# pikapuma/QuBLAS

Hardware: AMD Instinct MI355X
Metric: int-MAC/s (2*M*N*K/s) for Qgemul 4096^3 int<8,8>; % of MI355X int8 peak (higher is better)
Workload: dtype i8 limbs -> i32/i64; 1 GPU; 4096^3 Qgemul int<8,8> signed, linear class (MulArgs int17/frac16, AddArgs Qu<29,16>, C Qu<23,8>), 3x3 int8-limb MFMA; M_per_gpu=4096, N=4096, K=4096, class=linear

## Files before the change

include/qgemul.h:

```cpp
#ifndef QGEMUL_H_
#define QGEMUL_H_

#include <stddef.h>
#include <stdint.h>

#ifdef __cplusplus
extern "C" {
#endif

#define QGEMUL_ABI_VERSION 1u
#define QG_MAX_LEVELS 40

enum {
    QG_RND_POS_INF = 0,
    QG_RND_NEG_INF = 1,
    QG_RND_ZERO = 2,
    QG_RND_INF = 3,
    QG_RND_CONV = 4,
    QG_TRN_TCPL = 5,
    QG_TRN_SMGN = 6
};

enum {
    QG_SAT_TCPL = 0,
// ... 40 lines not shown
    int64_t M, N, K;
    qfmt a[2], b[2], c[2];
    qfmt mul[8];
    uint32_t n_levels;
    uint32_t reserved2;
    qfmt level_add[2][QG_MAX_LEVELS];
    qfmt level[2][QG_MAX_LEVELS];
} qgemul_desc;

typedef struct qgemul_opts {
    int64_t lda, ldb, ldc;
    int32_t device;
    uint32_t flags;
} qgemul_opts;

enum {
    QG_OPT_FORCE_TREE = 1u,
    QG_OPT_CHECK_RANGE = 2u,
    QG_OPT_GENERIC_TREE = 4u,
    QG_OPT_RUNTIME_MODES = 8u,
    QG_OPT_FUSED_EPILOGUE = 16u,
    QG_OPT_UNFUSED_EPILOGUE = 32u,
    QG_OPT_GENERIC_LAYOUT = 64u,
    QG_OPT_ARITHMETIC_CONV = 256u,
    QG_OPT_ALL_DEVICES = 512u,
    QG_OPT_BALANCED_LIMBS = 1024u,
    QG_OPT_LOCKSTEP_TILES = 128u
};

enum {
    QG_OK = 0,
    QG_EINVAL = -1,
    QG_EUNSUPPORTED = -2,
    QG_EHIP = -3,
    QG_ERCCL = -4,
    QG_ERANGE = -5,
    QG_ENOGPU = -6
};

enum {
    QG_CLASS_LINEAR = 1,
    QG_CLASS_TREE = 2
};

typedef struct qgemul_info {
    int32_t cls;
// ... 135 lines not shown
```

qublas_amd/build.py:

```python
from __future__ import annotations

import os
import subprocess
import sys

HERE = os.path.dirname(os.path.abspath(__file__))
CSRC = os.path.join(HERE, "csrc")
SOURCES = ["qg_api.hip", "qg_pack.hip", "qg_eltwise.hip", "qg_tree.hip", "qg_tree_fast.hip", "qg_tree64.hip", "qg_tree_cplx.hip", "qg_gemv.hip", "qg_mfma.hip", "qg_mfma_pp.hip", "qg_mfma_ppl.hip", "qg_comm.hip", "qg_plan.cpp"]
HEADERS = ["qg_ops.h", "qg_forms.h", "qg_plan.h", "qg_kernels.h", "qg_step_all.h", "qg_eltwise.h", "qg_eltwise_args.h", "qg_fix.h", os.path.join("..", "..", "include", "qgemul.h")]
LIB = os.path.join(HERE, "libqugemm.so")
LIB_DIAG = os.path.join(HERE, "libqugemm_diag.so")


def _stale(obj: str, deps) -> bool:
    if not os.path.exists(obj):
        return True
    t = os.path.getmtime(obj)
    return any(os.path.getmtime(d) > t for d in deps if os.path.exists(d))


def build(force: bool = False, verbose: bool = False, diag: bool = False) -> str:
    hipcc = os.environ.get("HIPCC", "/opt/rocm/bin/hipcc")
    hdrs = [os.path.join(CSRC, h) for h in HEADERS]
    objdir = os.path.join(HERE, "build", "diag") if diag else os.path.join(HERE, "build")
    LIB = LIB_DIAG if diag else globals()["LIB"]
    os.makedirs(objdir, exist_ok=True)
    objs = []
    procs = []
    for s in SOURCES:
        src = os.path.join(CSRC, s)
        obj = os.path.join(objdir, s.rsplit(".", 1)[0] + ".o")
# ... 21 lines not shown
```

qublas_amd/capi.py:

```python
from __future__ import annotations

import ctypes as C
import os
from typing import Optional

import numpy as np

from .desc import (Qcomplex, Qu, host_layout, qgemul_desc, qgemul_ep_args, qgemul_epilogue, qgemul_epilogue_cplx, qgemul_info,
                   qgemul_opts)

_HERE = os.path.dirname(os.path.abspath(__file__))
LIB_PATH = os.path.join(_HERE, "libqugemm_diag.so" if os.environ.get("QUBLAS_AMD_DIAG") == "1" else "libqugemm.so")

QG_OK, QG_EINVAL, QG_EUNSUPPORTED, QG_EHIP, QG_ERCCL, QG_ERANGE, QG_ENOGPU = 0, -1, -2, -3, -4, -5, -6
OPT_FORCE_TREE, OPT_CHECK_RANGE, OPT_GENERIC_TREE, OPT_RUNTIME_MODES, OPT_FUSED_EPILOGUE, OPT_UNFUSED_EPILOGUE = 1, 2, 4, 8, 16, 32
OPT_GENERIC_LAYOUT, OPT_LOCKSTEP_TILES, OPT_ARITHMETIC_CONV, OPT_ALL_DEVICES = 64, 128, 256, 512
OPT_BALANCED_LIMBS = 1024
OPERAND_A, OPERAND_B, OPERAND_C = 0, 1, 2
BITS_ASCII, BITS_PACKED = 0, 1
KERNEL_NAMES = {0: "none", 1: "mfma_i8", 2: "mfma_i8_limb", 3: "tree_i32", 4: "tree_i64", 5: "tree_cplx", 6: "tree_cplx_i32", 7: "mfma_cplx", 8: "gemv_i32", 9: "gemv_i64", 10: "tree_i128"}

EXPORTS = [
    "qgemul_classify", "qgemul_strerror", "qgemul_abi_version", "qgemul_last_hip_error", "qgemul_run",
    "qgemul_ctx_create", "qgemul_ctx_destroy", "qgemul_ctx_sync", "qgemul_ctx_stream",
    "qgemul_plan_create", "qgemul_plan_destroy", "qgemul_plan_info",
    "qgemul_dev_alloc", "qgemul_dev_free", "qgemul_memcpy_h2d", "qgemul_memcpy_d2h",
    "qgemul_pack", "qgemul_pack_f64", "qgemul_unpack_c", "qgemul_execute", "qgemul_fill_packed", "qgemul_time_execute",
    "qgemul_classify_ep", "qgemul_plan_create_ep", "qgemul_packed_e_bytes", "qgemul_pack_e", "qgemul_execute_ep",
    "qgemul_time_execute_ep", "qgemul_run_ep", "qgemul_plan_fuses_epilogue", "qgemul_plan_packed_layout", "qgemul_classify_epc", "qgemul_plan_create_epc", "qgemul_run_epc",
    "qgemul_bitstream_bytes", "qgemul_export_bitstream", "qgemul_run_release", "qgemul_run_sharded", "qgemul_execute_host_c", "qgemul_plan_stores_host_c",
    "qgemul_comm_unique_id", "qgemul_comm_create", "qgemul_comm_destroy", "qgemul_comm_info", "qgemul_gather_packed_c", "qgemul_comm_fence",
    "qgemul_comm_sync", "qgemul_comm_barrier", "qgemul_comm_max_f64", "qgemul_last_rccl_error", "qgemul_ctx_device",
]

_lib = None


class QgemulError(RuntimeError):
    def __init__(self, status: int, what: str = ""):
# ... 330 lines not shown
```

qublas_amd/csrc/qg_api.hip:

```cpp
#include <hip/hip_runtime.h>
#include <stdio.h>
#include <stdlib.h>
#include <string.h>

#include <new>

#include "../../include/qgemul.h"
#include "qg_kernels.h"
#include "qg_plan.h"

static thread_local int g_last_hip = 0;

#define QG_HIP(expr)                         \
    do {                                     \
        hipError_t e_ = (expr);              \
        if (e_ != hipSuccess) {              \
            g_last_hip = (int)e_;            \
            return QG_EHIP;                  \
        }                                    \
    } while (0)

struct qgemul_ctx {
    int device;
    hipStream_t stream;
// ... 242 lines not shown
        const bool pp_centred = cfg.variant && !ep && sbits(d->c) <= 31 && (tc.identity || (tc.d >= 0 && tc.W <= 30));
        if (cfg.variant && (int64_t)mn * d->K <= (1ll << 17) - 1 && !an->wide && !an->generic_only && !(centred && LA == 1 && LB == 1 && !pp_centred))
            kernel = d->is_complex ? QG_KERNEL_MFMA_CPLX : ((LA == 1 && LB == 1) ? QG_KERNEL_MFMA_I8 : QG_KERNEL_MFMA_I8_LIMB);
        else if (!d->is_complex && !(d->N == 1 && (an->gemv_ok || an->gemv_wide_ok) && !(flags & QG_OPT_GENERIC_TREE)) &&
                 comp_geometry(LA, LB, d, flags, &comp, &cfg)) {
            kernel = (LA == 1 && LB == 1) ? QG_KERNEL_MFMA_I8 : QG_KERNEL_MFMA_I8_LIMB;
            comp.wide = an->wide;
            snprintf(info->reason, sizeof info->reason, "linear class: %d k-chunk(s) x %d x %d limb groups on the MFMA kernels, exact %s combine", comp.nc, comp.ga, comp.gb,
                     comp.wide ? "128-bit" : "64-bit");
        } else {
            LA = LB = 0;
            centred = false;
            snprintf(info->reason, sizeof info->reason, "linear class, but limbs/K outside the MFMA kernels' range: tree kernel");
        }
    }
    pc->M = d->M;
    pc->N = d->N;
    pc->parts = parts;
    pc->cbytes = pow2_bytes(sbits(d->c));
    if (an->band && pc->cbytes < (hc->sb[0] > hc->sb[1] ? hc->sb[0] : hc->sb[1])) pc->cbytes = hc->sb[0] > hc->sb[1] ? hc->sb[0] : hc->sb[1];
    pc->ldc = d->M;
    pc->elem_bytes = hc->size;
    for (int p = 0; p < 2; ++p) { pc->off[p] = hc->off[p]; pc->sb[p] = hc->sb[p]; }
    if (kernel != QG_KERNEL_NONE) {
        *pa = QPackedGeom{round_up(d->M, cfg.TM), round_up(d->K, cfg.BK), 1, LA, cfg.TM, cfg.BK};
        *pb = QPackedGeom{round_up(d->N, cfg.TN), round_up(d->K, cfg.BK), 1, LB, cfg.TN, cfg.BK};
        if (comp.on) {
            pa->K_p = pb->K_p = round_up(comp.kc, cfg.BK);
            pa->limbs = comp.la[0];
            pb->limbs = comp.lb[0];
        }
        pc->Mp = pa->rows_p;
        pc->Np = pb->rows_p;
        pc->tm = cfg.TM;
        pc->tn = cfg.TN;
        if (d->is_complex) {
            pc->Mp = d->M;
            pc->Np = d->N;
            pc->tm = pc->tn = 0;
        }
    } else {
        const bool fast = !(flags & QG_OPT_GENERIC_TREE);
        const QTreeChoice tc = qg_tree_choice(an, d, flags, false);
        kernel = tc.kernel;
        if (kernel == QG_KERNEL_TREE_I128)
            snprintf(info->reason, sizeof info->reason, "exact tree evaluation on 128-bit values (intermediates of %d bits)", an->max_bits);
        if (kernel == QG_KERNEL_TREE_I32)
            snprintf(info->reason, sizeof info->reason, "exact tree evaluation; tree kernel steps: %s", qg_form_name(tc.tree));
        if (kernel == QG_KERNEL_GEMV_I64)
            snprintf(info->reason, sizeof info->reason, "exact tree evaluation; one-column kernel steps: run-time modes, 64-bit values");
        if (kernel == QG_KERNEL_GEMV_I32)
            snprintf(info->reason, sizeof info->reason, "exact tree evaluation; one-column kernel steps: %s", qg_form_name(tc.gemv));
        if (kernel == QG_KERNEL_TREE_CPLX_I32)
            snprintf(info->reason, sizeof info->reason, "exact tree evaluation; complex kernel steps: %s", qg_form_name(tc.cplx));
        const bool t64 = kernel == QG_KERNEL_TREE_I64 && an->tree64_ok && fast;
        const int64_t Kt = (kernel == QG_KERNEL_TREE_I32 || kernel == QG_KERNEL_TREE_CPLX_I32 || kernel == QG_KERNEL_GEMV_I32 || kernel == QG_KERNEL_GEMV_I64 || t64)
                               ? ((int64_t)1 << an->tree.n_levels_k) : d->K;
        *pa = QPackedGeom{d->M, Kt, info->in_bits[0] <= 32 ? 4 : 8, 0, 0, 0};
// ... 32 lines not shown
        pa->bias = -centreA;
        pb->bias = -centreB;
        pa->rowsum_off = round_up(info->packed_bytes[0], 256);
        pb->rowsum_off = round_up(info->packed_bytes[1], 256);
        info->packed_bytes[0] = pa->rowsum_off + pa->rows_p * 8;
        info->packed_bytes[1] = pb->rowsum_off + pb->rows_p * 8;
    }
    if (!comp.on && !centred) {
        static const bool no_kara = QG_DIAG_ENV("QG_NO_KARA");
        auto ubits = [](qfmt f) { return (int)f.I + (int)f.F + (f.S ? 1 : 0); };
        if (!no_kara && !d->is_complex && LA == 2 && LB == 2 && (kernel == QG_KERNEL_MFMA_I8_LIMB) && (cfg.variant == 3 || cfg.variant == 10) && ubits(d->a[0]) <= 12 &&
            ubits(d->b[0]) <= 12 && d->K * (int64_t)(126 * 126) < (1ll << 31)) {
            cfg.variant = 3;
            for (QPackedGeom* g : {pa, pb}) {
                const qfmt f = g == pa ? d->a[0] : d->b[0];
                g->digit6 = 1;
                g->bias = f.S ? ((int64_t)1 << ((int)f.I + (int)f.F)) : 0;
                g->rowsum_off = g->trailer + QG_TRAILER_BYTES;
            }
            info->packed_bytes[0] += pa->rows_p * 8;
            info->packed_bytes[1] += pb->rows_p * 8;
        }
    }
    info->packed_bytes[2] = (int64_t)parts * pc->Mp * pc->Np * pc->cbytes;
    *pLA = LA;
    *pLB = LB;
    *pVar = cfg;
    if (pc_c) *pc_c = *pc;
    if (ep && an->band) {
        info->supported = 0;
        snprintf(info->reason, sizeof info->reason, "element-wise chain after a plan whose C can leave its format (multi-word comparison artefact of the reference)");
        return QG_EUNSUPPORTED;
    }
    if (ep) {
        if ((d->is_complex != 0) != (ev->im != nullptr)) {
            info->supported = 0;
            snprintf(info->reason, sizeof info->reason, d->is_complex ? "complex GEMM: the chain is a qgemul_epilogue_cplx" : "real GEMM: the chain is a qgemul_epilogue");
            return QG_EINVAL;
        }
        QEpTable local[2];
        QEpTable* t[2] = {ept ? ept : &local[0], ept_im ? ept_im : &local[1]};
        qfmt df[2] = {ep->d, ep->d};
        for (int part = 0; part < parts; ++part) {
            const qgemul_epilogue* e = part ? ev->im : ep;
            int ep_bits = 0;
            char why[96];
// ... 420 lines not shown
    if (!p || !packed_dev || !dst_dev) return QG_EINVAL;
    QG_ON_DEVICE(p->ctx);
    QCGeom c = p->pc;
    c.ldc = ld ? ld : p->desc.M;
    QG_HIP(qg_launch_unpack_c(c, packed_dev, dst_dev, p->ctx->stream, (p->flags & QG_OPT_GENERIC_LAYOUT) ? 1 : 0));
    return QG_OK;
}

static int execute_kernel(qgemul_plan* p, void* packedC, const void* packedA, const void* packedB, const qgemul_ep_args* epa, const HostC* hostc = nullptr);

int qgemul_execute(qgemul_plan* p, void* packedC, const void* packedA, const void* packedB)
{
    if (!p || !packedC || !packedA || !packedB) return QG_EINVAL;
    if (p->has_ep) return QG_EINVAL;
    if (p->desc.M == 0 || p->desc.N == 0) return QG_OK;
    QG_ON_DEVICE(p->ctx);
    return execute_kernel(p, packedC, packedA, packedB, nullptr);
}

static bool stores_host_c(const qgemul_plan* p)
{
    if (p->has_ep || p->desc.is_complex || wide_epilogue(p) || p->comp.on) return false;
    if (p->info.kernel != QG_KERNEL_MFMA_I8 && p->info.kernel != QG_KERNEL_MFMA_I8_LIMB) return false;
    if (p->variant != 9 && p->variant != 10) return false;
    if (p->variant == 10 && (p->pa.rows_p / p->cfg.TM) * (p->pb.rows_p / p->cfg.TN) < 256) return false;
    return (p->pc.cbytes == 4 || p->pc.cbytes == 8) && p->pc.cbytes == p->hc.size;
}

int qgemul_plan_stores_host_c(const qgemul_plan* p) { return p && stores_host_c(p) ? 1 : 0; }

int qgemul_execute_host_c(qgemul_plan* p, void* C_dev, int64_t ldc, const void* packedA, const void* packedB)
{
    if (!p || !C_dev || !packedA || !packedB || p->has_ep) return QG_EINVAL;
    if (ldc && ldc < p->desc.M) return QG_EINVAL;
    if (p->desc.M == 0 || p->desc.N == 0) return QG_OK;
    QG_ON_DEVICE(p->ctx);
    if (stores_host_c(p)) {
        const HostC h{C_dev, ldc ? ldc : p->desc.M};
        return execute_kernel(p, C_dev, packedA, packedB, nullptr, &h);
    }
    if (!p->hostc_pc) QG_HIP(hipMalloc(&p->hostc_pc, (size_t)p->info.packed_bytes[2] ? (size_t)p->info.packed_bytes[2] : 16));
    const int st = execute_kernel(p, p->hostc_pc, packedA, packedB, nullptr);
    if (st != QG_OK) return st;
    QCGeom c = p->pc;
    c.ldc = ldc ? ldc : p->desc.M;
    QG_HIP(qg_launch_unpack_c(c, p->hostc_pc, C_dev, p->ctx->stream, (p->flags & QG_OPT_GENERIC_LAYOUT) ? 1 : 0));
    return QG_OK;
// ... 170 lines not shown
        memset(&a, 0, sizeof a);
        a.A = (const int8_t*)packedA;
        a.B = (const int8_t*)packedB;
        a.C = packedC;
        a.Mp = p->pa.rows_p;
        a.Np = p->pb.rows_p;
        a.Kp = p->pa.K_p;
        a.cbytes = pcg.cbytes;
        a.variant = p->variant;
        a.to_c = p->an.lin.to_c[0];
        a.maskA = p->pa.trailer ? (const uint32_t*)((const char*)packedA + p->pa.trailer) : nullptr;
        a.maskB = p->pb.trailer ? (const uint32_t*)((const char*)packedB + p->pb.trailer) : nullptr;
#ifdef QG_DIAG
        a.dbg = g_diag_stamps;
#endif
        centre_args(p, a, packedA, packedB);
        if (p->pa.digit6) {
            a.kara = 1;
            a.rsA = (const int64_t*)((const char*)packedA + p->pa.rowsum_off);
            a.rsB = (const int64_t*)((const char*)packedB + p->pb.rowsum_off);
            a.biasA = p->pa.bias;
            a.biasB = p->pb.bias;
            a.corr = p->desc.K * p->pa.bias * p->pb.bias;
        }
        if (wide_epilogue(p)) {
            a.C = p->wide_ws;
            a.cbytes = 4;
            memset(&a.to_c, 0, sizeof a.to_c);
            a.to_c.identity = 1;
            QG_HIP(qg_launch_mfma(p->LA, p->LB, a, st));
            QEltwiseArgs f;
            memset(&f, 0, sizeof f);
            f.C = (const char*)p->wide_ws;
            f.D = (char*)packedC;
            f.n = pcg.Mp * pcg.Np;
            f.cbytes = 4;
            f.t.dbytes = pcg.cbytes;
            f.t.to_d = p->an.lin.to_c[0];
            QG_HIP(qg_launch_eltwise(f, st));
            return QG_OK;
        }
        if (hostc) {
            a.C = hostc->C;
            a.c_host = 1;
            a.c_ld = hostc->ld;
            a.c_M = p->desc.M;
// ... 582 lines not shown
```

qublas_amd/csrc/qg_kernels.h:

```cpp
#pragma once
#include <hip/hip_runtime.h>
#include <stdint.h>
#include <stdlib.h>

#include <atomic>

#include "qg_eltwise_args.h"
#include "qg_plan.h"

struct QOperandGeom {
    int64_t rows, K;
    int64_t rs, ks;
    int32_t elem_bytes;
    int32_t off[2], sb[2];
    int32_t parts;
    int32_t W[2], S[2];
    int32_t F[2], Q[2], O[2];
    int64_t k0;
};

struct QPackedGeom {
    int64_t rows_p, K_p;
    int32_t cbytes;
    int32_t limbs;
// ... 80 lines not shown
hipError_t qg_launch_gemv(const QTreeTable* dev_table, int n_levels, int b_is_bit, QGemvForm form, const void* A, const void* B, void* C,
                          int64_t M, int64_t K, int cbytes, hipStream_t st, int wide = 0);

hipError_t qg_launch_tree_cplx_fast(const QTreeTable* dev_table, int n_levels, QCplxForm form, int tf, const void* A, const void* B, void* C,
                                    int64_t M, int64_t N, int64_t K, int cbytes, hipStream_t st);

struct QMfmaCfg {
    int variant;
    int TM, TN, BK;
};
QMfmaCfg qg_mfma_pick(int LA, int LB, int64_t M, int64_t N, uint32_t opt_flags = 0);
struct QMfmaArgs {
    const int8_t* A;
    const int8_t* B;
    void* C;
    int64_t Mp, Np, Kp;
    int32_t cbytes;
    int32_t variant;
    QStep to_c;
    const int64_t* rsA;
    const int64_t* rsB;
    int64_t biasA, biasB, corr;
    int32_t kara, pad3_;
    const uint32_t* maskA;
    const uint32_t* maskB;
    int32_t has_ep, pad_;
    uint32_t* dbg;
    int32_t c_host, c_vec;
    int64_t c_ld, c_M, c_N;
    QEpTable ep;
    QEpArgs epa;
};
hipError_t qg_launch_mfma(int LA, int LB, const QMfmaArgs& a, hipStream_t st);
hipError_t qg_launch_mfma_pp(const QMfmaArgs& a, hipStream_t st);
bool qg_mfma_ppl_applies(int LA, int LB, const QMfmaArgs& a);
hipError_t qg_launch_mfma_ppl(int limbs, const QMfmaArgs& a, hipStream_t st);

inline hipError_t qg_lds_attr(const void* fn, int bytes, std::atomic<uint64_t>& done)
{
    int dev = 0;
    hipError_t e = hipGetDevice(&dev);
    if (e != hipSuccess) return e;
    if (dev >= 0 && dev < 64 && ((done.load(std::memory_order_acquire) >> dev) & 1)) return hipSuccess;
    e = hipFuncSetAttribute(fn, hipFuncAttributeMaxDynamicSharedMemorySize, bytes);
    if (e == hipSuccess && dev >= 0 && dev < 64) done.fetch_or(1ull << dev, std::memory_order_release);
    return e;
}

#ifdef QG_DIAG
#define QG_DIAG_ENV(name) (getenv(name) != nullptr)
#else
#define QG_DIAG_ENV(name) false
#endif

hipError_t qg_launch_eltwise(const QEltwiseArgs& g, hipStream_t st);
hipError_t qg_launch_pack_e(const QCGeom& c, int part, const void* src, int64_t ld, int stride, int off, int src_bytes, void* dst, int ebytes,
                            hipStream_t st);

struct QBitsArgs {
// ... 16 lines not shown
```

qublas_amd/csrc/qg_mfma.hip:

```cpp
#include <hip/hip_runtime.h>
#include <stdlib.h>

#include <atomic>
#include <utility>

#include "qg_eltwise.h"
#include "qg_kernels.h"
#include "qg_step_all.h"

namespace {

typedef int v4i __attribute__((ext_vector_type(4)));
typedef int v16i __attribute__((ext_vector_type(16)));

#define QG_GLOBAL_PTR(p) ((const __attribute__((address_space(1))) void*)(p))
#define QG_LDS_PTR(p) ((__attribute__((address_space(3))) void*)(p))

template <int BK>
__device__ __forceinline__ int swz(int r)
{
    constexpr int CPR = BK / 16;
    constexpr int RPB = 256 / BK;
    const int q = (r / RPB) % CPR;
    return BK == 64 ? ((0x78 >> (2 * q)) & 3) : q;
// ... 718 lines not shown
    }
    {
        static const bool no_small = QG_DIAG_ENV("QG_NO_SMALL_TILES");
        const int64_t mid = ((M + 127) / 128) * ((N + 127) / 128);
        if (((LA == 3 && LB == 3) || (LA == 2 && LB == 2)) && mid >= 256 && !(opt_flags & QG_OPT_LOCKSTEP_TILES)) return QMfmaCfg{10, 128, 128, 64};
        if (!no_small && mid <= 128 && ((M + 63) / 64) * ((N + 63) / 64) > mid) return QMfmaCfg{6, 64, 64, 64};
    }
    return QMfmaCfg{3, 128, 128, 64};
}

#ifdef QG_DIAG
static int ablation()
{
    static int v = -1;
    if (v < 0) { const char* e = getenv("QG_ABLATE"); v = e ? atoi(e) : 0; }
    return v;
}
#else
static constexpr int ablation() { return 0; }
#endif

hipError_t qg_launch_mfma(int LA, int LB, const QMfmaArgs& a_in, hipStream_t st)
{
    if (a_in.variant == 10 && qg_mfma_ppl_applies(LA, LB, a_in)) return qg_launch_mfma_ppl(LA, a_in, st);
    QMfmaArgs a_v3;
    if (a_in.variant == 10) { a_v3 = a_in; a_v3.variant = 3; }
    const QMfmaArgs& a = a_in.variant == 10 ? a_v3 : a_in;
#ifdef QG_DIAG
    if (const int abl = ablation(); abl > 0 && abl < 16) {
        if (LA == 3 && LB == 3 && a.variant == 3) {
            switch (abl) {
            case 1: return launch<3, 3, 64, 2, 4, 2, 1, 3, 1>(a, st);
            case 2: return launch<3, 3, 64, 2, 4, 2, 1, 3, 2>(a, st);
            case 3: return launch<3, 3, 64, 2, 4, 2, 1, 3, 3>(a, st);
            case 4: return launch<3, 3, 64, 2, 4, 2, 1, 3, 4>(a, st);
            case 6: return launch<3, 3, 64, 2, 4, 2, 1, 3, 6>(a, st);
            case 15: return launch<3, 3, 64, 2, 4, 2, 1, 3, 15>(a, st);
            default: return launch<3, 3, 64, 2, 4, 2, 1, 3, 5>(a, st);
            }
        }
        if (LA == 1 && LB == 1 && a.variant == 2) {
            switch (abl) {
            case 1: return launch<1, 1, 64, 2, 4, 4, 2, 3, 1>(a, st);
            case 2: return launch<1, 1, 64, 2, 4, 4, 2, 3, 2>(a, st);
            case 3: return launch<1, 1, 64, 2, 4, 4, 2, 3, 3>(a, st);
            case 4: return launch<1, 1, 64, 2, 4, 4, 2, 3, 4>(a, st);
// ... 84 lines not shown
```

qublas_amd/csrc/qg_pack.hip:

```cpp
#include <hip/hip_runtime.h>

#include <type_traits>

#include "qg_kernels.h"

namespace {

__device__ __forceinline__ int64_t load_host_part(const char* src, int64_t e, int elem_bytes, int off, int sb)
{
    const char* p = src + e * elem_bytes + off;
    return sb == 4 ? (int64_t)(*(const int32_t*)p) : *(const int64_t*)p;
}

__device__ __forceinline__ void store_container(char* dst, int64_t idx, int cbytes, int64_t v)
{
    switch (cbytes) {
    case 1: ((int8_t*)dst)[idx] = (int8_t)v; break;
    case 2: ((int16_t*)dst)[idx] = (int16_t)v; break;
    case 4: ((int32_t*)dst)[idx] = (int32_t)v; break;
    default: ((int64_t*)dst)[idx] = v; break;
    }
}

__device__ __forceinline__ int64_t load_container(const char* src, int64_t idx, int cbytes)
// ... 48 lines not shown
        if (p.digit6) {
            for (int l = 0; l < p.limbs; ++l) {
                ((int8_t*)dst)[((blk + l) * p.tr + rl) * p.bk + slot * 16 + (kl & 15)] = (int8_t)(v & 63);
                v >>= 6;
            }
            return 0;
        }
        for (int l = 0; l < p.limb0; ++l) v = (v - (int64_t)(int8_t)(v & 0xff)) >> 8;
        for (int l = 0; l < p.limbs; ++l) {
            int64_t d = (int64_t)(int8_t)(v & 0xff);
            ((int8_t*)dst)[((blk + l) * p.tr + rl) * p.bk + slot * 16 + (kl & 15)] = (int8_t)d;
            mask |= d ? (1u << l) : 0u;
            v = (v - d) >> 8;
        }
    }
    return mask;
}

template <bool R_FAST, bool VEC = false, bool F64 = false>
__global__ __launch_bounds__(256) void k_pack_limb32(QOperandGeom g, QPackedGeom p, const int32_t* __restrict__ src, int8_t* __restrict__ dst,
                                                     int check, int* flag)
{
    const int kt = (int)(p.K_p / 64);
    const int64_t nblk = (int64_t)kt * (p.rows_p / 64);
    const int t = threadIdx.x;
    const int row_l = R_FAST ? (t & 63) : (t >> 2), kc = R_FAST ? (t >> 6) : (t & 3);
    const int W = g.W[0];
    const int64_t lo = g.S[0] ? -((int64_t)1 << W) : 0, hi = ((int64_t)1 << W) - 1;
    unsigned mask = 0;
    bool bad = false;
    __shared__ unsigned long long rs_sh[64];
    for (int64_t blk_id = blockIdx.x; blk_id < nblk; blk_id += gridDim.x) {
    const int tk = (int)(blk_id % kt), tr64 = (int)(blk_id / kt);
    const int64_t r = (int64_t)tr64 * 64 + row_l, k0 = (int64_t)tk * 64 + kc * 16;
    int32_t v[16];
    const bool row_in = r < g.rows;
    const int32_t* q = src + r * g.rs + (k0 + g.k0) * g.ks;
    if constexpr (F64) {
        const double* qd = (const double*)src + r * g.rs + (k0 + g.k0) * g.ks;
        if (VEC && row_in && k0 + 16 <= g.K) {
            const double2* q2 = (const double2*)qd;
#pragma unroll
            for (int j = 0; j < 8; ++j) {
                const double2 x = q2[j];
                v[2 * j] = (int32_t)quantize_f64(x.x, W, g.S[0], g.F[0], g.Q[0], g.O[0]);
                v[2 * j + 1] = (int32_t)quantize_f64(x.y, W, g.S[0], g.F[0], g.Q[0], g.O[0]);
            }
        } else {
#pragma unroll
            for (int j = 0; j < 16; ++j)
                v[j] = (row_in && k0 + j < g.K) ? (int32_t)quantize_f64(qd[(int64_t)j * g.ks], W, g.S[0], g.F[0], g.Q[0], g.O[0]) : 0;
        }
    } else
    if (VEC && row_in && k0 + 16 <= g.K) {
        const int4* q4 = (const int4*)q;
#pragma unroll
        for (int j = 0; j < 4; ++j) {
            const int4 x = q4[j];
            v[4 * j] = x.x; v[4 * j + 1] = x.y; v[4 * j + 2] = x.z; v[4 * j + 3] = x.w;
        }
#pragma unroll
        for (int j = 0; j < 16; ++j) bad |= (v[j] < lo) | (v[j] > hi);
    } else {
#pragma unroll
        for (int j = 0; j < 16; ++j) {
            v[j] = (row_in && k0 + j < g.K) ? q[(int64_t)j * g.ks] : 0;
            bad |= (v[j] < lo) | (v[j] > hi);
        }
    }
    if (p.offs) {
        const int32_t bias = (int32_t)p.bias;
        long long part = 0;
#pragma unroll
        for (int j = 0; j < 16; ++j) {
            if (row_in && k0 + j < g.K) v[j] += bias;
            part += v[j];
        }
        if (p.offs != 3) {
            __syncthreads();
            if (t < 64) rs_sh[t] = 0;
            __syncthreads();
            if (part) atomicAdd(&rs_sh[row_l], (unsigned long long)part);
            __syncthreads();
            if (t < 64 && rs_sh[t] && (int64_t)tr64 * 64 + t < p.rows_p)
                atomicAdd((unsigned long long*)((char*)dst + p.rowsum_off) + (int64_t)tr64 * 64 + t, rs_sh[t]);
        }
    }
    const int rl = (int)(r % p.tr);
    const int sw = p.bk == 64 ? (0x78 >> (2 * ((rl >> 2) & 3))) & 3 : (rl >> 1) & 7;
    const int c = p.bk == 64 ? kc : (tk & 1) * 4 + kc;
    const int64_t blk = ((r / p.tr) * (p.K_p / p.bk) + (p.bk == 64 ? tk : tk >> 1)) * p.limbs;
    int8_t* out = dst + (blk * p.tr + rl) * p.bk + ((c ^ sw) * 16);
    for (int l = 0; l < p.limb0; ++l)
#pragma unroll
        for (int j = 0; j < 16; ++j) v[j] = (int32_t)(((int64_t)v[j] - (int32_t)(int8_t)(v[j] & 0xff)) >> 8);
    for (int l = 0; l < p.limbs; ++l) {
        uint32_t w[4] = {0, 0, 0, 0};
        uint32_t any = 0;
#pragma unroll
        for (int j = 0; j < 16; ++j) {
            const int32_t d = (int32_t)(int8_t)(v[j] & 0xff);
            w[j >> 2] |= (uint32_t)(d & 0xff) << (8 * (j & 3));
            any |= (uint32_t)d;
            v[j] = (int32_t)(((int64_t)v[j] - d) >> 8);
        }
        *(uint4*)(out + (int64_t)l * p.tr * p.bk) = make_uint4(w[0], w[1], w[2], w[3]);
        mask |= any ? (1u << l) : 0u;
    }
    }
    if (p.trailer) {
        __shared__ unsigned wmask[4];
#pragma unroll
        for (int o = 32; o; o >>= 1) mask |= __shfl_xor(mask, o);
        if ((t & 63) == 0) wmask[t >> 6] = mask;
        __syncthreads();
        if (t == 0) {
            const unsigned m = wmask[0] | wmask[1] | wmask[2] | wmask[3];
            if (m) atomicOr((unsigned*)(dst + p.trailer) + (blockIdx.x & (QG_MASK_WORDS - 1)), m);
// ... 306 lines not shown
    if (n <= 0) return hipSuccess;
    hipLaunchKernelGGL(k_cplx_combine, dim3((unsigned)((n + 255) / 256)), dim3(256), 0, st, g);
    return hipGetLastError();
}

static hipError_t zero_trailer(const QPackedGeom& p, void* dst, hipStream_t st)
{
    if (p.offs == 1)
        if (hipError_t e = hipMemsetAsync((char*)dst + p.rowsum_off, 0, (size_t)p.rows_p * 8, st); e != hipSuccess) return e;
    if (!p.trailer) return hipSuccess;
    const size_t bytes = QG_TRAILER_BYTES + (p.digit6 ? (size_t)p.rows_p * 8 : 0);
    return hipMemsetAsync((char*)dst + p.trailer, 0, bytes, st);
}

hipError_t qg_launch_pack(const QOperandGeom& g, const QPackedGeom& p, const void* src, void* dst, int check_range,
                          int* range_flag, hipStream_t st, int generic)
{
    int64_t blocks = ((p.K_p + 63) / 64) * ((p.rows_p + 63) / 64) * g.parts;
    if (blocks <= 0) return hipSuccess;
    if (blocks > 0x7fffffffll) return hipErrorInvalidValue;
    if (hipError_t e = zero_trailer(p, dst, st); e != hipSuccess) return e;
    const bool no_fast = generic != 0;
    const bool centred_fast = !p.offs || (g.W[0] <= 24 && p.bias > -(1ll << 24) && p.bias < (1ll << 24));
    if (!no_fast && g.parts == 1 && g.elem_bytes == 4 && g.sb[0] == 4 && g.off[0] == 0 && p.limbs >= 1 && p.limbs <= 3 && !p.digit6 && centred_fast && (p.bk == 64 || p.bk == 128) &&
        p.tr % 64 == 0 && p.rows_p % p.tr == 0 && p.K_p % p.bk == 0 && g.W[0] <= 30 && ((uintptr_t)src & 3) == 0 && ((uintptr_t)dst & 15) == 0) {
        const int64_t nblk = (p.K_p / 64) * (p.rows_p / 64);
        const unsigned nb = (unsigned)(nblk < 2048 ? nblk : 2048);
        if (g.rs == 1 && g.ks != 1) hipLaunchKernelGGL(k_pack_limb32<true>, dim3(nb), dim3(256), 0, st, g, p, (const int32_t*)src, (int8_t*)dst, check_range, range_flag);
        else if (g.ks == 1 && g.rs % 4 == 0 && g.k0 % 4 == 0 && ((uintptr_t)src & 15) == 0)
            hipLaunchKernelGGL((k_pack_limb32<false, true>), dim3(nb), dim3(256), 0, st, g, p, (const int32_t*)src, (int8_t*)dst, check_range, range_flag);
        else hipLaunchKernelGGL(k_pack_limb32<false>, dim3(nb), dim3(256), 0, st, g, p, (const int32_t*)src, (int8_t*)dst, check_range, range_flag);
        return hipGetLastError();
    }
    hipLaunchKernelGGL(k_pack, dim3((unsigned)blocks), dim3(256), 0, st, g, p, (const char*)src, (char*)dst, check_range,
                       range_flag, 0, 0ull, 0);
    return hipGetLastError();
}

hipError_t qg_launch_pack_f64(const QOperandGeom& g, const QPackedGeom& p, const void* src, void* dst, hipStream_t st, int generic)
{
    int64_t blocks = ((p.K_p + 63) / 64) * ((p.rows_p + 63) / 64) * g.parts;
    if (blocks <= 0) return hipSuccess;
    if (blocks > 0x7fffffffll) return hipErrorInvalidValue;
    if (hipError_t e = zero_trailer(p, dst, st); e != hipSuccess) return e;
    const bool centred_fast = !p.offs || (g.W[0] <= 24 && p.bias > -(1ll << 24) && p.bias < (1ll << 24));
    if (!generic && g.parts == 1 && p.limbs >= 1 && p.limbs <= 3 && !p.digit6 && centred_fast && (p.bk == 64 || p.bk == 128) && p.tr % 64 == 0 && p.rows_p % p.tr == 0 &&
        p.K_p % p.bk == 0 && g.W[0] <= 30 && ((uintptr_t)src & 7) == 0 && ((uintptr_t)dst & 15) == 0) {
        const int64_t nblk = (p.K_p / 64) * (p.rows_p / 64);
        const unsigned nb = (unsigned)(nblk < 2048 ? nblk : 2048);
        if (g.rs == 1 && g.ks != 1) hipLaunchKernelGGL((k_pack_limb32<true, false, true>), dim3(nb), dim3(256), 0, st, g, p, (const int32_t*)src, (int8_t*)dst, 0, (int*)nullptr);
        else if (g.ks == 1 && g.rs % 2 == 0 && g.k0 % 2 == 0 && ((uintptr_t)src & 15) == 0)
            hipLaunchKernelGGL((k_pack_limb32<false, true, true>), dim3(nb), dim3(256), 0, st, g, p, (const int32_t*)src, (int8_t*)dst, 0, (int*)nullptr);
        else hipLaunchKernelGGL((k_pack_limb32<false, false, true>), dim3(nb), dim3(256), 0, st, g, p, (const int32_t*)src, (int8_t*)dst, 0, (int*)nullptr);
        return hipGetLastError();
    }
    hipLaunchKernelGGL(k_pack, dim3((unsigned)blocks), dim3(256), 0, st, g, p, (const char*)src, (char*)dst, 0, (int*)nullptr, 2, 0ull, 0);
    return hipGetLastError();
}

hipError_t qg_launch_fill(const QOperandGeom& g, const QPackedGeom& p, uint64_t seed, int dist, void* dst, hipStream_t st)
{
    int64_t blocks = ((p.K_p + 63) / 64) * ((p.rows_p + 63) / 64) * g.parts;
    if (blocks <= 0) return hipSuccess;
    if (blocks > 0x7fffffffll) return hipErrorInvalidValue;
    if (hipError_t e = zero_trailer(p, dst, st); e != hipSuccess) return e;
    hipLaunchKernelGGL(k_pack, dim3((unsigned)blocks), dim3(256), 0, st, g, p, (const char*)nullptr, (char*)dst, 0,
                       (int*)nullptr, 1, seed, dist);
    return hipGetLastError();
}

hipError_t qg_launch_unpack_c(const QCGeom& c, const void* packed, void* dst, hipStream_t st, int generic)
// ... 23 lines not shown
```

qublas_amd/profmeta.py:

```python
from __future__ import annotations

import hashlib
import json
import os
import subprocess

ROOT = os.path.dirname(os.path.dirname(os.path.abspath(__file__)))
CSRC = os.path.join(ROOT, "qublas_amd", "csrc")
KERNELS_JSON = os.path.join(ROOT, "profiles", "kernels.json")

COMMON = ["qg_ops.h", "qg_kernels.h"]
FAMILY_SOURCES = {
    "mfma_i8": ["qg_mfma.hip", "qg_mfma_pp.hip", "qg_step_all.h"],
    "mfma_i8_limb": ["qg_mfma.hip", "qg_mfma_ppl.hip", "qg_step_all.h"],
    "mfma_cplx": ["qg_mfma.hip", "qg_mfma_ppl.hip", "qg_step_all.h", "qg_pack.hip"],
    "tree_i32": ["qg_tree_fast.hip", "qg_fix.h", "qg_forms.h"],
    "tree_i64": ["qg_tree64.hip", "qg_tree.hip"],
    "tree_i128": ["qg_tree.hip"],
    "tree_cplx": ["qg_tree.hip"],
    "tree_cplx_i32": ["qg_tree_cplx.hip", "qg_fix.h", "qg_forms.h"],
    "gemv_i32": ["qg_gemv.hip", "qg_fix.h", "qg_forms.h"],
    "gemv_i64": ["qg_gemv.hip", "qg_fix.h", "qg_forms.h"],
}


def source_hashes(engine_kernel: str) -> dict:
    out = {}
    for f in FAMILY_SOURCES.get(engine_kernel, []) + COMMON:
        p = os.path.join(CSRC, f)
        out[f] = hashlib.sha256(open(p, "rb").read()).hexdigest()[:16] if os.path.exists(p) else None
    return out


def git_head() -> str:
    try:
        return subprocess.check_output(["git", "-C", ROOT, "rev-parse", "--short", "HEAD"], text=True, stderr=subprocess.DEVNULL).strip()
    except Exception:
# ... 25 lines not shown
```

Before: 370800 billion int-op/s (2*M*N*K/s).

## Add Karatsuba base-64 three-digit limb kernel using six MFMA products

Adds a new MFMA kernel that splits each biased 17-18 bit operand into three unsigned base-64 digits and forms the product with a three-way Karatsuba scheme: six digit products instead of the nine products of the balanced base-256 limb path. Digit sums are computed in registers before the extra MFMAs, and results are recombined in 64-bit arithmetic with bias and row-sum corrections. The kernel uses 96x128 tiles, triple-buffered LDS loads and a persistent tiled grid, and packing gains a digit6 mode. The aim is to cut matrix-core work by about a third, at the cost of extra LDS traffic, register pressure, recombination work, and a constraint on K so the digit sums cannot overflow int32.

```diff
diff --git a/include/qgemul.h b/include/qgemul.h
--- a/include/qgemul.h
+++ b/include/qgemul.h
@@ -86,6 +86,7 @@
     QG_OPT_FUSED_EPILOGUE = 16u,
     QG_OPT_UNFUSED_EPILOGUE = 32u,
     QG_OPT_GENERIC_LAYOUT = 64u,
+    QG_OPT_SCHOOLBOOK_LIMBS = 2048u,
     QG_OPT_ARITHMETIC_CONV = 256u,
     QG_OPT_ALL_DEVICES = 512u,
     QG_OPT_BALANCED_LIMBS = 1024u,
diff --git a/qublas_amd/build.py b/qublas_amd/build.py
--- a/qublas_amd/build.py
+++ b/qublas_amd/build.py
@@ -6,7 +6,7 @@
 
 HERE = os.path.dirname(os.path.abspath(__file__))
 CSRC = os.path.join(HERE, "csrc")
-SOURCES = ["qg_api.hip", "qg_pack.hip", "qg_eltwise.hip", "qg_tree.hip", "qg_tree_fast.hip", "qg_tree64.hip", "qg_tree_cplx.hip", "qg_gemv.hip", "qg_mfma.hip", "qg_mfma_pp.hip", "qg_mfma_ppl.hip", "qg_comm.hip", "qg_plan.cpp"]
+SOURCES = ["qg_api.hip", "qg_pack.hip", "qg_eltwise.hip", "qg_tree.hip", "qg_tree_fast.hip", "qg_tree64.hip", "qg_tree_cplx.hip", "qg_gemv.hip", "qg_mfma.hip", "qg_mfma_pp.hip", "qg_mfma_ppl.hip", "qg_mfma_k6.hip", "qg_comm.hip", "qg_plan.cpp"]
 HEADERS = ["qg_ops.h", "qg_forms.h", "qg_plan.h", "qg_kernels.h", "qg_step_all.h", "qg_eltwise.h", "qg_eltwise_args.h", "qg_fix.h", os.path.join("..", "..", "include", "qgemul.h")]
 LIB = os.path.join(HERE, "libqugemm.so")
 LIB_DIAG = os.path.join(HERE, "libqugemm_diag.so")
diff --git a/qublas_amd/capi.py b/qublas_amd/capi.py
--- a/qublas_amd/capi.py
+++ b/qublas_amd/capi.py
@@ -15,6 +15,7 @@
 QG_OK, QG_EINVAL, QG_EUNSUPPORTED, QG_EHIP, QG_ERCCL, QG_ERANGE, QG_ENOGPU = 0, -1, -2, -3, -4, -5, -6
 OPT_FORCE_TREE, OPT_CHECK_RANGE, OPT_GENERIC_TREE, OPT_RUNTIME_MODES, OPT_FUSED_EPILOGUE, OPT_UNFUSED_EPILOGUE = 1, 2, 4, 8, 16, 32
 OPT_GENERIC_LAYOUT, OPT_LOCKSTEP_TILES, OPT_ARITHMETIC_CONV, OPT_ALL_DEVICES = 64, 128, 256, 512
+OPT_SCHOOLBOOK_LIMBS = 2048
 OPT_BALANCED_LIMBS = 1024
 OPERAND_A, OPERAND_B, OPERAND_C = 0, 1, 2
 BITS_ASCII, BITS_PACKED = 0, 1
diff --git a/qublas_amd/csrc/qg_api.hip b/qublas_amd/csrc/qg_api.hip
--- a/qublas_amd/csrc/qg_api.hip
+++ b/qublas_amd/csrc/qg_api.hip
@@ -288,6 +288,16 @@
     pc->ldc = d->M;
     pc->elem_bytes = hc->size;
     for (int p = 0; p < 2; ++p) { pc->off[p] = hc->off[p]; pc->sb[p] = hc->sb[p]; }
+    bool k6 = false, ppl33 = false;
+    {
+        static const bool no_kara3 = QG_DIAG_ENV("QG_NO_KARA3");
+        auto ubits = [](qfmt f) { return (int)f.I + (int)f.F + (f.S ? 1 : 0); };
+        const int cb = pow2_bytes(sbits(d->c));
+        ppl33 = kernel == QG_KERNEL_MFMA_I8_LIMB && !comp.on && !d->is_complex && !ep && LA == 3 && LB == 3 && cfg.variant == 10 && (cb == 4 || cb == 8);
+        k6 = ppl33 && !no_kara3 && !(flags & QG_OPT_SCHOOLBOOK_LIMBS) && !centred && !an->band && ubits(d->a[0]) >= 13 && ubits(d->a[0]) <= 18 &&
+             ubits(d->b[0]) >= 13 && ubits(d->b[0]) <= 18 && d->K * (int64_t)(126 * 126) < (1ll << 31);
+        if (k6) cfg = QMfmaCfg{QG_K6_VARIANT, QG_K6_TM, QG_K6_TN, QG_K6_BK};
+    }
     if (kernel != QG_KERNEL_NONE) {
         *pa = QPackedGeom{round_up(d->M, cfg.TM), round_up(d->K, cfg.BK), 1, LA, cfg.TM, cfg.BK};
         *pb = QPackedGeom{round_up(d->N, cfg.TN), round_up(d->K, cfg.BK), 1, LB, cfg.TN, cfg.BK};
@@ -300,6 +310,10 @@
         pc->Np = pb->rows_p;
         pc->tm = cfg.TM;
         pc->tn = cfg.TN;
+        if (k6) {
+            pc->Mp = round_up(d->M, 128);
+            pc->tm = 128;
+        }
         if (d->is_complex) {
             pc->Mp = d->M;
             pc->Np = d->N;
@@ -378,6 +392,19 @@
             info->packed_bytes[1] += pb->rows_p * 8;
         }
     }
+    if (k6) {
+        for (QPackedGeom* g : {pa, pb}) {
+            const qfmt f = g == pa ? d->a[0] : d->b[0];
+            g->digit6 = 1;
+            g->bias = f.S ? ((int64_t)1 << ((int)f.I + (int)f.F)) : 0;
+            g->rowsum_off = g->trailer + QG_TRAILER_BYTES;
+        }
+        info->packed_bytes[0] += pa->rows_p * 8;
+        info->packed_bytes[1] += pb->rows_p * 8;
+        snprintf(info->reason, sizeof info->reason, "linear class: three base-64 digits per operand, six products (two-group kernel, 96x128 tiles)");
+    } else if (ppl33) {
+        snprintf(info->reason, sizeof info->reason, "linear class: balanced base-256 limbs, nine products (two-group kernel, 128x128 tiles)");
+    }
     info->packed_bytes[2] = (int64_t)parts * pc->Mp * pc->Np * pc->cbytes;
     *pLA = LA;
     *pLB = LB;
@@ -844,7 +871,7 @@
 {
     if (p->has_ep || p->desc.is_complex || wide_epilogue(p) || p->comp.on) return false;
     if (p->info.kernel != QG_KERNEL_MFMA_I8 && p->info.kernel != QG_KERNEL_MFMA_I8_LIMB) return false;
-    if (p->variant != 9 && p->variant != 10) return false;
+    if (p->variant != 9 && p->variant != 10 && p->variant != QG_K6_VARIANT) return false;
     if (p->variant == 10 && (p->pa.rows_p / p->cfg.TM) * (p->pb.rows_p / p->cfg.TN) < 256) return false;
     return (p->pc.cbytes == 4 || p->pc.cbytes == 8) && p->pc.cbytes == p->hc.size;
 }
@@ -1061,6 +1088,7 @@
             a.biasA = p->pa.bias;
             a.biasB = p->pb.bias;
             a.corr = p->desc.K * p->pa.bias * p->pb.bias;
+            a.Mc = pcg.Mp;
         }
         if (wide_epilogue(p)) {
             a.C = p->wide_ws;
diff --git a/qublas_amd/csrc/qg_kernels.h b/qublas_amd/csrc/qg_kernels.h
--- a/qublas_amd/csrc/qg_kernels.h
+++ b/qublas_amd/csrc/qg_kernels.h
@@ -126,6 +126,7 @@
     const int64_t* rsB;
     int64_t biasA, biasB, corr;
     int32_t kara, pad3_;
+    int64_t Mc;
     const uint32_t* maskA;
     const uint32_t* maskB;
     int32_t has_ep, pad_;
@@ -139,6 +140,9 @@
 hipError_t qg_launch_mfma_pp(const QMfmaArgs& a, hipStream_t st);
 bool qg_mfma_ppl_applies(int LA, int LB, const QMfmaArgs& a);
 hipError_t qg_launch_mfma_ppl(int limbs, const QMfmaArgs& a, hipStream_t st);
+enum { QG_K6_VARIANT = 11, QG_K6_TM = 96, QG_K6_TN = 128, QG_K6_BK = 64 };
+bool qg_mfma_k6_applies(const QMfmaArgs& a);
+hipError_t qg_launch_mfma_k6(const QMfmaArgs& a, hipStream_t st);
 
 inline hipError_t qg_lds_attr(const void* fn, int bytes, std::atomic<uint64_t>& done)
 {
diff --git a/qublas_amd/csrc/qg_mfma.hip b/qublas_amd/csrc/qg_mfma.hip
--- a/qublas_amd/csrc/qg_mfma.hip
+++ b/qublas_amd/csrc/qg_mfma.hip
@@ -764,6 +764,7 @@
 
 hipError_t qg_launch_mfma(int LA, int LB, const QMfmaArgs& a_in, hipStream_t st)
 {
+    if (a_in.variant == QG_K6_VARIANT) return qg_launch_mfma_k6(a_in, st);
     if (a_in.variant == 10 && qg_mfma_ppl_applies(LA, LB, a_in)) return qg_launch_mfma_ppl(LA, a_in, st);
     QMfmaArgs a_v3;
     if (a_in.variant == 10) { a_v3 = a_in; a_v3.variant = 3; }
diff --git a/qublas_amd/csrc/qg_mfma_k6.hip b/qublas_amd/csrc/qg_mfma_k6.hip
--- /dev/null
+++ b/qublas_amd/csrc/qg_mfma_k6.hip
@@ -0,0 +1,278 @@
+#include <hip/hip_runtime.h>
+
+#include <atomic>
+#include <type_traits>
+
+#include "qg_kernels.h"
+#include "qg_step_all.h"
+
+namespace {
+
+typedef int v4i __attribute__((ext_vector_type(4)));
+
+#define QG_GLOBAL_PTR(p) ((const __attribute__((address_space(1))) void*)(p))
+#define QG_LDS_PTR(p) ((__attribute__((address_space(3))) void*)(p))
+
+constexpr int TM = 96, TN = 128, BK = 64;
+constexpr int PLANE_A = TM * BK, PLANE_B = TN * BK;
+constexpr int BUF = 3 * PLANE_A + 3 * PLANE_B;
+constexpr int NBUF = 3;
+
+__device__ __forceinline__ void tile_of(int w, int tiles_m, int tiles_n, int& tile_m, int& tile_n)
+{
+    constexpr int GM = 8;
+    const int grp = w / (GM * tiles_n);
+    const int first_m = grp * GM;
+    const int gsz = (tiles_m - first_m) < GM ? (tiles_m - first_m) : GM;
+    const int rem = w - grp * (GM * tiles_n);
+    tile_m = first_m + rem % gsz;
+    tile_n = rem / gsz;
+}
+
+template <bool FAST, int CB>
+__global__ __launch_bounds__(512) void k_mfma_k6(QMfmaArgs g)
+{
+    extern __shared__ __attribute__((aligned(16))) char smem[];
+    const int lane = threadIdx.x & 63;
+    const int wave = __builtin_amdgcn_readfirstlane(threadIdx.x >> 6);
+    const int wm = wave >> 2, wn = wave & 3;
+
+    const int tiles_m = (int)(g.Mp / TM), tiles_n = (int)(g.Np / TN);
+    const int nwg = tiles_m * tiles_n;
+    int w_first, w_step, n_my;
+    {
+        const int q = nwg / 8, r = nwg % 8, x = blockIdx.x % 8;
+        const int start = x < r ? x * (q + 1) : r * (q + 1) + (x - r) * q;
+        const int cnt = q + (x < r ? 1 : 0), j = blockIdx.x / 8, P = gridDim.x / 8;
+        w_first = start + j;
+        w_step = P;
+        n_my = j < cnt ? (cnt - j + P - 1) / P : 0;
+    }
+    if (n_my == 0) return;
+
+    const int nk = (int)(g.Kp / BK);
+    const int64_t panel_a = (int64_t)nk * 3 * PLANE_A, panel_b = (int64_t)nk * 3 * PLANE_B;
+    const uint32_t lane16 = (uint32_t)(lane * 16);
+    const int pa0 = wave * 1024, pa1 = (8 + wave) * 1024, pa2 = 16 * 1024 + wave * 256;
+    const int pb0 = wave * 1024, pb1 = (8 + wave) * 1024, pb2 = (16 + wave) * 1024;
+    struct Cursor { const int8_t* a; const int8_t* b; int kt, ti; };
+    auto cursor_at_tile = [&](int ti) {
+        int tm, tn;
+        tile_of(w_first + ti * w_step, tiles_m, tiles_n, tm, tn);
+        return Cursor{g.A + tm * panel_a, g.B + tn * panel_b, 0, ti};
+    };
+    auto advance = [&](Cursor c) {
+        if (c.kt + 1 < nk) return Cursor{c.a + 3 * PLANE_A, c.b + 3 * PLANE_B, c.kt + 1, c.ti};
+        if (c.ti + 1 < n_my) return cursor_at_tile(c.ti + 1);
+        return c;
+    };
+    auto issue_a = [&](int buf_off, int piece, const Cursor& c) {
+        __builtin_amdgcn_global_load_lds(QG_GLOBAL_PTR(c.a + piece + lane16), QG_LDS_PTR(smem + buf_off + piece), 16, 0, 0);
+    };
+    auto issue_b = [&](int buf_off, int piece, const Cursor& c) {
+        __builtin_amdgcn_global_load_lds(QG_GLOBAL_PTR(c.b + piece + lane16), QG_LDS_PTR(smem + buf_off + 3 * PLANE_A + piece), 16, 0, 0);
+    };
+    auto issue_tile = [&](int buf_off, const Cursor& c) {
+        issue_b(buf_off, pb0, c);
+        issue_a(buf_off, pa0, c);
+        issue_b(buf_off, pb1, c);
+        issue_a(buf_off, pa1, c);
+        issue_b(buf_off, pb2, c);
+        __builtin_amdgcn_global_load_lds(QG_GLOBAL_PTR(c.a + pa2 + lane * 4), QG_LDS_PTR(smem + buf_off + pa2), 4, 0, 0);
+    };
+
+    enum { S00, S11, P01, S22, P12, P02, NACC };
+    v4i acc[NACC][3][2];
+    const int fr = lane & 15, fq = lane >> 4;
+    const int chunk = (fq ^ ((0x78 >> (2 * (fr >> 2))) & 3)) * 16;
+    const int a_lane = (wm * 48 + fr) * BK + chunk;
+    const int b_lane = 3 * PLANE_A + (wn * 32 + fr) * BK + chunk;
+    v4i fa[3][3], fb[3][2];
+    auto read_ab = [&](int buf_off, int plane, int set) {
+#pragma unroll
+        for (int i = 0; i < 3; ++i) fa[set][i] = *(const v4i*)(smem + buf_off + plane * PLANE_A + i * (16 * BK) + a_lane);
+#pragma unroll
+        for (int j = 0; j < 2; ++j) fb[set][j] = *(const v4i*)(smem + buf_off + plane * PLANE_B + j * (16 * BK) + b_lane);
+    };
+    auto product = [&](int s, int set) {
+#pragma unroll
+        for (int i = 0; i < 3; ++i)
+#pragma unroll
+            for (int j = 0; j < 2; ++j) acc[s][i][j] = __builtin_amdgcn_mfma_i32_16x16x64_i8(fa[set][i], fb[set][j], acc[s][i][j], 0, 0, 0);
+    };
+#define QG_LOAD_DONE(WAIT)                                          \
+    do {                                                            \
+        WAIT;                                                       \
+        asm volatile("s_waitcnt lgkmcnt(0)" ::: "memory");          \
+        __builtin_amdgcn_sched_barrier(0);                          \
+        __builtin_amdgcn_s_barrier();                               \
+        __builtin_amdgcn_sched_barrier(0);                          \
+    } while (0)
+#define QG_MFMA_DONE()                                              \
+    do {                                                            \
+        __builtin_amdgcn_s_setprio(0);                              \
+        __builtin_amdgcn_sched_barrier(0);                          \
+        __builtin_amdgcn_s_barrier();                               \
+        __builtin_amdgcn_sched_barrier(0);                          \
+    } while (0)
+
+    Cursor nxt = cursor_at_tile(0);
+    issue_tile(0, nxt);
+    nxt = advance(nxt);
+    issue_tile(BUF, nxt);
+    nxt = advance(nxt);
+    asm volatile("s_waitcnt vmcnt(6)" ::: "memory");
+    __builtin_amdgcn_s_barrier();
+    asm volatile("" ::: "memory");
+
+    int cur = 0, fill = 2 * BUF;
+    for (int ti = 0; ti < n_my; ++ti) {
+#pragma unroll
+        for (int s = 0; s < NACC; ++s)
+#pragma unroll
+            for (int i = 0; i < 3; ++i)
+#pragma unroll
+                for (int j = 0; j < 2; ++j)
+#pragma unroll
+                    for (int e = 0; e < 4; ++e) acc[s][i][j][e] = 0;
+        if (wm == 1) __builtin_amdgcn_s_barrier();
+        __builtin_amdgcn_sched_barrier(0);
+
+        for (int kt = 0; kt < nk; ++kt) {
+            read_ab(cur, 0, 0);
+            read_ab(cur, 1, 1);
+            read_ab(cur, 2, 2);
+            issue_tile(fill, nxt);
+            QG_LOAD_DONE(asm volatile("s_waitcnt vmcnt(6)" ::: "memory"));
+            __builtin_amdgcn_s_setprio(1);
+            product(S00, 0);
+            product(S11, 1);
+            product(S22, 2);
+#pragma unroll
+            for (int i = 0; i < 3; ++i) fa[1][i] += fa[2][i];
+#pragma unroll
+            for (int j = 0; j < 2; ++j) fb[1][j] += fb[2][j];
+            product(P12, 1);
+#pragma unroll
+            for (int i = 0; i < 3; ++i) fa[1][i] = fa[1][i] + fa[0][i] - fa[2][i];
+#pragma unroll
+            for (int j = 0; j < 2; ++j) fb[1][j] = fb[1][j] + fb[0][j] - fb[2][j];
+            product(P01, 1);
+#pragma unroll
+            for (int i = 0; i < 3; ++i) fa[0][i] += fa[2][i];
+#pragma unroll
+            for (int j = 0; j < 2; ++j) fb[0][j] += fb[2][j];
+            product(P02, 0);
+            QG_MFMA_DONE();
+            nxt = advance(nxt);
+            const int t = cur;
+            cur = cur + BUF == NBUF * BUF ? 0 : cur + BUF;
+            fill = t;
+        }
+        if (wm == 0) __builtin_amdgcn_s_barrier();
+        __builtin_amdgcn_sched_barrier(0);
+
+        int tile_m, tile_n;
+        tile_of(w_first + ti * w_step, tiles_m, tiles_n, tile_m, tile_n);
+        const QStep st = g.to_c;
+        char* C = (char*)g.C;
+        constexpr int CT = 128;
+        [[maybe_unused]] const int sh = st.d;
+#pragma unroll
+        for (int i = 0; i < 3; ++i) {
+            int64_t s[8];
+#pragma unroll
+            for (int j = 0; j < 2; ++j)
+#pragma unroll
+                for (int e = 0; e < 4; ++e) {
+                    const int64_t s00 = acc[S00][i][j][e], s11 = acc[S11][i][j][e], s22 = acc[S22][i][j][e];
+                    const int64_t c1 = (int64_t)acc[P01][i][j][e] - s00 - s11, c2 = (int64_t)acc[P02][i][j][e] - s00 - s22 + s11,
+                                  c3 = (int64_t)acc[P12][i][j][e] - s11 - s22;
+                    const int64_t x = s00 + (c1 << 6) + (c2 << 12) + (c3 << 18) + (s22 << 24);
+                    s[j * 4 + e] = (int64_t)((uint64_t)x + (uint64_t)g.corr - (uint64_t)g.biasA * (uint64_t)g.rsB[(int64_t)tile_n * TN + wn * 32 + j * 16 + fr] -
+                                             (uint64_t)g.biasB * (uint64_t)g.rsA[(int64_t)tile_m * TM + wm * 48 + i * 16 + 4 * fq + e]);
+                }
+            if constexpr (FAST) {
+#pragma unroll
+                for (int o = 0; o < 8; ++o) {
+                    const int64_t x = s[o] >> sh, y = x < st.lo ? st.lo : x;
+                    s[o] = y > st.hi ? st.hi : y;
+                }
+            } else {
+                qg_step_all<int64_t, 8>(s, st);
+            }
+            const int row0 = wm * 48 + i * 16 + 4 * fq;
+#pragma unroll
+            for (int j = 0; j < 2; ++j) {
+                const int col = wn * 32 + j * 16 + fr;
+                const int64_t* q = s + j * 4;
+                if (g.c_host) {
+                    const int64_t gr = (int64_t)tile_m * TM + row0, gc = (int64_t)tile_n * TN + col;
+                    if (gc < g.c_N) {
+                        using E = std::conditional_t<CB == 4, int32_t, int64_t>;
+                        E* dst = (E*)C + gc * g.c_ld + gr;
+                        if (gr + 3 < g.c_M && g.c_vec) {
+                            if constexpr (CB == 4) *(int4*)dst = make_int4((int)q[0], (int)q[1], (int)q[2], (int)q[3]);
+                            else { *(longlong2*)dst = make_longlong2(q[0], q[1]); *(longlong2*)(dst + 2) = make_longlong2(q[2], q[3]); }
+                        } else {
+#pragma unroll
+                            for (int e = 0; e < 4; ++e)
+                                if (gr + e < g.c_M) dst[e] = (E)q[e];
+                        }
+                    }
+                    continue;
+                }
+                const int64_t gr = (int64_t)tile_m * TM + row0;
+                if (gr >= g.Mc) continue;
+                const int64_t base = (((gr / CT) * tiles_n + tile_n) * CT + col) * CT + gr % CT;
+                if constexpr (CB == 4) {
+                    *(int4*)(C + base * 4) = make_int4((int)q[0], (int)q[1], (int)q[2], (int)q[3]);
+                } else {
+                    int64_t* p = (int64_t*)(C + base * 8);
+                    *(longlong2*)p = make_longlong2(q[0], q[1]);
+                    *(longlong2*)(p + 2) = make_longlong2(q[2], q[3]);
+                }
+            }
+        }
+    }
+    asm volatile("s_waitcnt vmcnt(0)" ::: "memory");
+#undef QG_LOAD_DONE
+#undef QG_MFMA_DONE
+}
+
+template <bool FAST, int CB>
+hipError_t launch_k6(const QMfmaArgs& a, unsigned grid, hipStream_t st)
+{
+    constexpr int lds = NBUF * BUF;
+    static std::atomic<uint64_t> attr_done{0};
+    if (hipError_t e = qg_lds_attr((const void*)k_mfma_k6<FAST, CB>, lds, attr_done); e != hipSuccess) return e;
+    hipLaunchKernelGGL((k_mfma_k6<FAST, CB>), dim3(grid), dim3(512), lds, st, a);
+    return hipGetLastError();
+}
+
+}
+
+bool qg_mfma_k6_applies(const QMfmaArgs& a)
+{
+    if (a.has_ep || !a.kara || a.variant != 11 || !a.rsA || !a.rsB) return false;
+    if (a.cbytes != 4 && a.cbytes != 8) return false;
+    return a.Kp > 0 && a.Kp % BK == 0 && a.Mp % TM == 0 && a.Np % TN == 0 && a.Mc > 0 && a.Mc % 128 == 0 && a.Mc <= a.Mp + 127;
+}
+
+hipError_t qg_launch_mfma_k6(const QMfmaArgs& a, hipStream_t st)
+{
+    if (!qg_mfma_k6_applies(a)) return hipErrorInvalidValue;
+    const int64_t blocks = (a.Mp / TM) * (a.Np / TN);
+    if (blocks <= 0) return hipSuccess;
+    if (blocks > 0x7fffffffll) return hipErrorInvalidValue;
+    int dev = 0, cus = 0;
+    if (hipError_t e = hipGetDevice(&dev); e != hipSuccess) return e;
+    if (hipError_t e = hipDeviceGetAttribute(&cus, hipDeviceAttributeMultiprocessorCount, dev); e != hipSuccess) return e;
+    int64_t grid = cus / 8 * 8;
+    if (grid < 8) grid = 8;
+    if (grid > blocks) grid = (blocks + 7) / 8 * 8;
+    const QStep& q = a.to_c;
+    const bool fast = !q.identity && q.O == QG_SAT_TCPL && q.Q == QG_TRN_TCPL && q.d >= 0;
+    if (a.cbytes == 4) return fast ? launch_k6<true, 4>(a, grid, st) : launch_k6<false, 4>(a, grid, st);
+    return fast ? launch_k6<true, 8>(a, grid, st) : launch_k6<false, 8>(a, grid, st);
+}
diff --git a/qublas_amd/csrc/qg_pack.hip b/qublas_amd/csrc/qg_pack.hip
--- a/qublas_amd/csrc/qg_pack.hip
+++ b/qublas_amd/csrc/qg_pack.hip
@@ -94,7 +94,7 @@
                                                      int check, int* flag)
 {
     const int kt = (int)(p.K_p / 64);
-    const int64_t nblk = (int64_t)kt * (p.rows_p / 64);
+    const int64_t nblk = (int64_t)kt * ((p.rows_p + 63) / 64);
     const int t = threadIdx.x;
     const int row_l = R_FAST ? (t & 63) : (t >> 2), kc = R_FAST ? (t >> 6) : (t & 3);
     const int W = g.W[0];
@@ -140,12 +140,13 @@
             bad |= (v[j] < lo) | (v[j] > hi);
         }
     }
-    if (p.offs) {
+    if (p.offs || p.digit6) {
         const int32_t bias = (int32_t)p.bias;
         long long part = 0;
 #pragma unroll
         for (int j = 0; j < 16; ++j) {
             if (row_in && k0 + j < g.K) v[j] += bias;
+            if (p.digit6) v[j] &= (1 << 18) - 1;
             part += v[j];
         }
         if (p.offs != 3) {
@@ -166,6 +167,19 @@
     for (int l = 0; l < p.limb0; ++l)
 #pragma unroll
         for (int j = 0; j < 16; ++j) v[j] = (int32_t)(((int64_t)v[j] - (int32_t)(int8_t)(v[j] & 0xff)) >> 8);
+    if (r >= p.rows_p) continue;
+    if (p.digit6) {
+        for (int l = 0; l < p.limbs; ++l) {
+            uint32_t w[4] = {0, 0, 0, 0};
+#pragma unroll
+            for (int j = 0; j < 16; ++j) {
+                w[j >> 2] |= (uint32_t)(v[j] & 63) << (8 * (j & 3));
+                v[j] >>= 6;
+            }
+            *(uint4*)(out + (int64_t)l * p.tr * p.bk) = make_uint4(w[0], w[1], w[2], w[3]);
+        }
+        continue;
+    }
     for (int l = 0; l < p.limbs; ++l) {
         uint32_t w[4] = {0, 0, 0, 0};
         uint32_t any = 0;
@@ -518,9 +532,9 @@
     if (hipError_t e = zero_trailer(p, dst, st); e != hipSuccess) return e;
     const bool no_fast = generic != 0;
     const bool centred_fast = !p.offs || (g.W[0] <= 24 && p.bias > -(1ll << 24) && p.bias < (1ll << 24));
-    if (!no_fast && g.parts == 1 && g.elem_bytes == 4 && g.sb[0] == 4 && g.off[0] == 0 && p.limbs >= 1 && p.limbs <= 3 && !p.digit6 && centred_fast && (p.bk == 64 || p.bk == 128) &&
-        p.tr % 64 == 0 && p.rows_p % p.tr == 0 && p.K_p % p.bk == 0 && g.W[0] <= 30 && ((uintptr_t)src & 3) == 0 && ((uintptr_t)dst & 15) == 0) {
-        const int64_t nblk = (p.K_p / 64) * (p.rows_p / 64);
+    if (!no_fast && g.parts == 1 && g.elem_bytes == 4 && g.sb[0] == 4 && g.off[0] == 0 && p.limbs >= 1 && p.limbs <= 3 && (!p.digit6 || p.limbs == 3) && centred_fast && (p.bk == 64 || p.bk == 128) &&
+        (p.tr % 64 == 0 || (p.digit6 && p.tr % 16 == 0)) && p.rows_p % p.tr == 0 && p.K_p % p.bk == 0 && g.W[0] <= 30 && ((uintptr_t)src & 3) == 0 && ((uintptr_t)dst & 15) == 0) {
+        const int64_t nblk = (p.K_p / 64) * ((p.rows_p + 63) / 64);
         const unsigned nb = (unsigned)(nblk < 2048 ? nblk : 2048);
         if (g.rs == 1 && g.ks != 1) hipLaunchKernelGGL(k_pack_limb32<true>, dim3(nb), dim3(256), 0, st, g, p, (const int32_t*)src, (int8_t*)dst, check_range, range_flag);
         else if (g.ks == 1 && g.rs % 4 == 0 && g.k0 % 4 == 0 && ((uintptr_t)src & 15) == 0)
@@ -540,9 +554,10 @@
     if (blocks > 0x7fffffffll) return hipErrorInvalidValue;
     if (hipError_t e = zero_trailer(p, dst, st); e != hipSuccess) return e;
     const bool centred_fast = !p.offs || (g.W[0] <= 24 && p.bias > -(1ll << 24) && p.bias < (1ll << 24));
-    if (!generic && g.parts == 1 && p.limbs >= 1 && p.limbs <= 3 && !p.digit6 && centred_fast && (p.bk == 64 || p.bk == 128) && p.tr % 64 == 0 && p.rows_p % p.tr == 0 &&
+    if (!generic && g.parts == 1 && p.limbs >= 1 && p.limbs <= 3 && (!p.digit6 || p.limbs == 3) && centred_fast && (p.bk == 64 || p.bk == 128) &&
+        (p.tr % 64 == 0 || (p.digit6 && p.tr % 16 == 0)) && p.rows_p % p.tr == 0 &&
         p.K_p % p.bk == 0 && g.W[0] <= 30 && ((uintptr_t)src & 7) == 0 && ((uintptr_t)dst & 15) == 0) {
-        const int64_t nblk = (p.K_p / 64) * (p.rows_p / 64);
+        const int64_t nblk = (p.K_p / 64) * ((p.rows_p + 63) / 64);
         const unsigned nb = (unsigned)(nblk < 2048 ? nblk : 2048);
         if (g.rs == 1 && g.ks != 1) hipLaunchKernelGGL((k_pack_limb32<true, false, true>), dim3(nb), dim3(256), 0, st, g, p, (const int32_t*)src, (int8_t*)dst, 0, (int*)nullptr);
         else if (g.ks == 1 && g.rs % 2 == 0 && g.k0 % 2 == 0 && ((uintptr_t)src & 15) == 0)
diff --git a/qublas_amd/profmeta.py b/qublas_amd/profmeta.py
--- a/qublas_amd/profmeta.py
+++ b/qublas_amd/profmeta.py
@@ -12,7 +12,7 @@
 COMMON = ["qg_ops.h", "qg_kernels.h"]
 FAMILY_SOURCES = {
     "mfma_i8": ["qg_mfma.hip", "qg_mfma_pp.hip", "qg_step_all.h"],
-    "mfma_i8_limb": ["qg_mfma.hip", "qg_mfma_ppl.hip", "qg_step_all.h"],
+    "mfma_i8_limb": ["qg_mfma.hip", "qg_mfma_ppl.hip", "qg_mfma_k6.hip", "qg_step_all.h"],
     "mfma_cplx": ["qg_mfma.hip", "qg_mfma_ppl.hip", "qg_step_all.h", "qg_pack.hip"],
     "tree_i32": ["qg_tree_fast.hip", "qg_fix.h", "qg_forms.h"],
     "tree_i64": ["qg_tree64.hip", "qg_tree.hip"],
```

Result: faster. 419600 billion int-op/s (2*M*N*K/s) (median of 6 runs) (+13.2%).
